# facebook/winterfell

Measured on NVIDIA H100. Metric: prover_ms, lower is better.
Workload: dtype u64

## Files before the change

winterfell_b200/csrc/gl64.cuh:

```cuda
#pragma once
#ifdef __CUDACC_RTC__
typedef unsigned long long uint64_t;
typedef unsigned int uint32_t;
typedef unsigned char uint8_t;
#else
#include <stdint.h>
#endif

#ifdef __CUDACC__
#define GL_HD __host__ __device__ __forceinline__
#else
#define GL_HD inline
#endif

typedef uint64_t u64;
typedef uint32_t u32;
typedef uint8_t u8;

#define GL_P 0xffffffff00000001ULL
#define GL_EPS 0xffffffffULL
#define GL_GENERATOR 7ULL
#define GL_TWO_ADIC_ROOT 7277203076849721926ULL

static inline u64 gl_add_host(u64 a, u64 b) {
    u64 r = a + b;
    if (r < a || r >= GL_P) r += GL_EPS;
    return r;
}
static inline u64 gl_sub_host(u64 a, u64 b) {
    u64 r = a - b;
    if (a < b) r -= GL_EPS;
    return r;
}
static inline u64 gl_reduce128_host(u64 lo, u64 hi) {
    u64 hh = hi >> 32, hl = hi & GL_EPS;
    u64 t = lo - hh;
    if (lo < hh) t -= GL_EPS;
    u64 m = (hl << 32) - hl;
    u64 r = t + m;
    if (r < m) r += GL_EPS;
    if (r >= GL_P) r -= GL_P;
    return r;
}

#if defined(__CUDACC__) && !defined(GL_LITERAL_EPS)
static __constant__ u32 GL_EPS_CONST = 0xffffffffu;
#define GL_EPS_OPERAND , "r"(GL_EPS_CONST)
#define GL_EPSM(n) "%" #n
#else
#define GL_EPS_OPERAND
#define GL_EPSM(n) "0xffffffff"
#endif
#ifdef __CUDA_ARCH__
__device__ __forceinline__ u64 gl_sub(u64 a, u64 b) {
    u64 r;
    asm("{\n\t"
        ".reg .u32 a0, a1, b0, b1, m;\n\t"
        "mov.b64 {a0, a1}, %1;\n\t"
        "mov.b64 {b0, b1}, %2;\n\t"
        "sub.cc.u32 a0, a0, b0;\n\t"
        "subc.cc.u32 a1, a1, b1;\n\t"
        "subc.u32 m, 0, 0;\n\t"
        "sub.cc.u32 a0, a0, m;\n\t"
        "subc.u32 a1, a1, 0;\n\t"
        "mov.b64 %0, {a0, a1};\n\t"
        "}"
        : "=l"(r)
        : "l"(a), "l"(b));
    return r;
}
__device__ __forceinline__ u64 gl_add(u64 a, u64 b) {
    u64 r;
    asm("{\n\t"
        ".reg .u32 a0, a1, b0, b1, m;\n\t"
        "mov.b64 {a0, a1}, %1;\n\t"
        "mov.b64 {b0, b1}, %2;\n\t"
        "sub.cc.u32 b0, 1, b0;\n\t"
        "subc.u32 b1, 0xffffffff, b1;\n\t"
        "sub.cc.u32 a0, a0, b0;\n\t"
        "subc.cc.u32 a1, a1, b1;\n\t"
        "subc.u32 m, 0, 0;\n\t"
        "sub.cc.u32 a0, a0, m;\n\t"
        "subc.u32 a1, a1, 0;\n\t"
        "mov.b64 %0, {a0, a1};\n\t"
        "}"
        : "=l"(r)
        : "l"(a), "l"(b));
    return r;
}
__device__ __forceinline__ void gl_butterfly(u64& a, u64& b) {
    u64 s, d;
    asm("{\n\t"
        ".reg .u32 a0, a1, b0, b1, n0, n1, s0, s1, m;\n\t"
        "mov.b64 {a0, a1}, %2;\n\t"
        "mov.b64 {b0, b1}, %3;\n\t"
        "sub.cc.u32 n0, 1, b0;\n\t"
        "subc.u32 n1, 0xffffffff, b1;\n\t"
        "sub.cc.u32 s0, a0, n0;\n\t"
        "subc.cc.u32 s1, a1, n1;\n\t"
        "subc.u32 m, 0, 0;\n\t"
        "sub.cc.u32 s0, s0, m;\n\t"
        "subc.u32 s1, s1, 0;\n\t"
        "mov.b64 %0, {s0, s1};\n\t"
        "sub.cc.u32 a0, a0, b0;\n\t"
        "subc.cc.u32 a1, a1, b1;\n\t"
        "subc.u32 m, 0, 0;\n\t"
        "sub.cc.u32 a0, a0, m;\n\t"
        "subc.u32 a1, a1, 0;\n\t"
        "mov.b64 %1, {a0, a1};\n\t"
        "}"
        : "=l"(s), "=l"(d)
        : "l"(a), "l"(b));
    a = s;
    b = d;
}
__device__ __forceinline__ u64 gl_canon(u64 r) {
    u64 o;
    asm("{\n\t"
        ".reg .u32 r0, r1, t0, t1, k;\n\t"
        "mov.b64 {r0, r1}, %1;\n\t"
        "add.cc.u32 t0, r0, 0xffffffff;\n\t"
        "addc.cc.u32 t1, r1, 0;\n\t"
        "addc.u32 k, 0, 0;\n\t"
        "sub.u32 r0, r0, k;\n\t"
        "add.u32 r1, r1, k;\n\t"
        "mov.b64 %0, {r0, r1};\n\t"
        "}"
        : "=l"(o)
        : "l"(r));
    return o;
}
__device__ __forceinline__ u64 gl_reduce128(u64 lo, u64 hi) {
    u64 r;
    asm("{\n\t"
        ".reg .u32 c0, c1, c2, c3, k, m, t0, t1;\n\t"
        "mov.b64 {c0, c1}, %1;\n\t"
        "mov.b64 {c2, c3}, %2;\n\t"
        "sub.cc.u32 c0, c0, c3;\n\t"
        "subc.cc.u32 c1, c1, 0;\n\t"
        "subc.u32 m, 0, 0;\n\t"
        "sub.cc.u32 c0, c0, m;\n\t"
        "subc.u32 c1, c1, 0;\n\t"
        "mad.lo.cc.u32 c0, c2, " GL_EPSM(3) ", c0;\n\t"
        "madc.hi.cc.u32 c1, c2, " GL_EPSM(3) ", c1;\n\t"
        "addc.u32 k, 0, 0;\n\t"
        "add.cc.u32 t0, c0, 0xffffffff;\n\t"
        "addc.cc.u32 t1, c1, 0;\n\t"
        "addc.u32 k, k, 0;\n\t"
        "mad.lo.cc.u32 c0, k, " GL_EPSM(3) ", c0;\n\t"
        "madc.hi.u32 c1, k, " GL_EPSM(3) ", c1;\n\t"
        "mov.b64 %0, {c0, c1};\n\t"
        "}"
        : "=l"(r)
        : "l"(lo), "l"(hi) GL_EPS_OPERAND);
    return r;
}
__device__ __forceinline__ u64 gl_mul(u64 a, u64 b) {
    u64 r;
    asm("{\n\t"
        ".reg .u32 a0, a1, b0, b1, c0, c1, c2, c3, o0, o1, o2, k, m, t0, t1;\n\t"
        "mov.b64 {a0, a1}, %1;\n\t"
        "mov.b64 {b0, b1}, %2;\n\t"
        "mul.lo.u32 c0, a0, b0;\n\t"
        "mul.hi.u32 c1, a0, b0;\n\t"
        "mul.lo.u32 c2, a1, b1;\n\t"
        "mul.hi.u32 c3, a1, b1;\n\t"
        "mul.lo.u32 o0, a0, b1;\n\t"
        "mul.hi.u32 o1, a0, b1;\n\t"
        "mad.lo.cc.u32 o0, a1, b0, o0;\n\t"
        "madc.hi.cc.u32 o1, a1, b0, o1;\n\t"
        "addc.u32 o2, 0, 0;\n\t"
        "add.cc.u32 c1, c1, o0;\n\t"
        "addc.cc.u32 c2, c2, o1;\n\t"
        "addc.u32 c3, c3, o2;\n\t"
        "sub.cc.u32 c0, c0, c3;\n\t"
        "subc.cc.u32 c1, c1, 0;\n\t"
        "subc.u32 m, 0, 0;\n\t"
        "sub.cc.u32 c0, c0, m;\n\t"
        "subc.u32 c1, c1, 0;\n\t"
        "mad.lo.cc.u32 c0, c2, " GL_EPSM(3) ", c0;\n\t"
        "madc.hi.cc.u32 c1, c2, " GL_EPSM(3) ", c1;\n\t"
        "addc.u32 k, 0, 0;\n\t"
        "add.cc.u32 t0, c0, 0xffffffff;\n\t"
        "addc.cc.u32 t1, c1, 0;\n\t"
        "addc.u32 k, k, 0;\n\t"
        "mad.lo.cc.u32 c0, k, " GL_EPSM(3) ", c0;\n\t"
        "madc.hi.u32 c1, k, " GL_EPSM(3) ", c1;\n\t"
        "mov.b64 %0, {c0, c1};\n\t"
        "}"
        : "=l"(r)
        : "l"(a), "l"(b) GL_EPS_OPERAND);
    return r;
}
__device__ __forceinline__ u64 gl_mul_weak(u64 a, u64 b) {
    u64 r;
    asm("{\n\t"
        ".reg .u32 a0, a1, b0, b1, c0, c1, c2, c3, o0, o1, o2, k, m;\n\t"
        "mov.b64 {a0, a1}, %1;\n\t"
        "mov.b64 {b0, b1}, %2;\n\t"
        "mul.lo.u32 c0, a0, b0;\n\t"
        "mul.hi.u32 c1, a0, b0;\n\t"
        "mul.lo.u32 c2, a1, b1;\n\t"
        "mul.hi.u32 c3, a1, b1;\n\t"
        "mul.lo.u32 o0, a0, b1;\n\t"
        "mul.hi.u32 o1, a0, b1;\n\t"
        "mad.lo.cc.u32 o0, a1, b0, o0;\n\t"
        "madc.hi.cc.u32 o1, a1, b0, o1;\n\t"
        "addc.u32 o2, 0, 0;\n\t"
        "add.cc.u32 c1, c1, o0;\n\t"
        "addc.cc.u32 c2, c2, o1;\n\t"
        "addc.u32 c3, c3, o2;\n\t"
        "sub.cc.u32 c0, c0, c3;\n\t"
        "subc.cc.u32 c1, c1, 0;\n\t"
        "subc.u32 m, 0, 0;\n\t"
        "sub.cc.u32 c0, c0, m;\n\t"
        "subc.u32 c1, c1, 0;\n\t"
        "mad.lo.cc.u32 c0, c2, " GL_EPSM(3) ", c0;\n\t"
        "madc.hi.cc.u32 c1, c2, " GL_EPSM(3) ", c1;\n\t"
        "addc.u32 k, 0, 0;\n\t"
        "mad.lo.cc.u32 c0, k, " GL_EPSM(3) ", c0;\n\t"
        "madc.hi.u32 c1, k, " GL_EPSM(3) ", c1;\n\t"
        "mov.b64 %0, {c0, c1};\n\t"
        "}"
        : "=l"(r)
        : "l"(a), "l"(b) GL_EPS_OPERAND);
    return r;
}
__device__ __forceinline__ u64 gl_sqr_weak(u64 a) {
    u64 r;
    asm("{\n\t"
        ".reg .u32 a0, a1, c0, c1, c2, c3, o0, o1, o2, k, m;\n\t"
        ".reg .u64 w;\n\t"
        "mov.b64 {a0, a1}, %1;\n\t"
        "mul.wide.u32 w, a0, a0;\n\t"
        "mov.b64 {c0, c1}, w;\n\t"
        "mul.wide.u32 w, a1, a1;\n\t"
        "mov.b64 {c2, c3}, w;\n\t"
        "mul.wide.u32 w, a0, a1;\n\t"
        "mov.b64 {o0, o1}, w;\n\t"
        "add.cc.u32 o0, o0, o0;\n\t"
        "addc.cc.u32 o1, o1, o1;\n\t"
        "addc.u32 o2, 0, 0;\n\t"
        "add.cc.u32 c1, c1, o0;\n\t"
        "addc.cc.u32 c2, c2, o1;\n\t"
        "addc.u32 c3, c3, o2;\n\t"
        "sub.cc.u32 c0, c0, c3;\n\t"
        "subc.cc.u32 c1, c1, 0;\n\t"
        "subc.u32 m, 0, 0;\n\t"
        "sub.cc.u32 c0, c0, m;\n\t"
        "subc.u32 c1, c1, 0;\n\t"
        "mad.lo.cc.u32 c0, c2, " GL_EPSM(2) ", c0;\n\t"
        "madc.hi.cc.u32 c1, c2, " GL_EPSM(2) ", c1;\n\t"
        "addc.u32 k, 0, 0;\n\t"
        "mad.lo.cc.u32 c0, k, " GL_EPSM(2) ", c0;\n\t"
        "madc.hi.u32 c1, k, " GL_EPSM(2) ", c1;\n\t"
        "mov.b64 %0, {c0, c1};\n\t"
        "}"
        : "=l"(r)
        : "l"(a) GL_EPS_OPERAND);
    return r;
}
template <int K>
__device__ __forceinline__ u64 gl_shl_dev(u64 x) {
    constexpr int R = K & 31;
    const u32 x0 = (u32)x, x1 = (u32)(x >> 32);
    const u32 y0 = x0 << R, y1 = R ? __funnelshift_l(x0, x1, R) : x1, y2 = R ? (x1 >> ((32 - R) & 31)) : 0;
    u64 o;
    if (K < 32) {
        asm("{\n\t"
            ".reg .u32 r0, r1, k, t0, t1;\n\t"
            "mad.lo.cc.u32 r0, %3, " GL_EPSM(4) ", %1;\n\t"
            "madc.hi.cc.u32 r1, %3, " GL_EPSM(4) ", %2;\n\t"
            "addc.u32 k, 0, 0;\n\t"
            "add.cc.u32 t0, r0, 0xffffffff;\n\t"
            "addc.cc.u32 t1, r1, 0;\n\t"
            "addc.u32 k, k, 0;\n\t"
            "mad.lo.cc.u32 r0, k, " GL_EPSM(4) ", r0;\n\t"
            "madc.hi.u32 r1, k, " GL_EPSM(4) ", r1;\n\t"
            "mov.b64 %0, {r0, r1};\n\t"
            "}" : "=l"(o) : "r"(y0), "r"(y1), "r"(y2) GL_EPS_OPERAND);
    } else if (K < 64) {
        asm("{\n\t"
            ".reg .u32 r0, r1, k, m, t0, t1;\n\t"
            "sub.cc.u32 r0, 0, %3;\n\t"
            "subc.cc.u32 r1, %1, 0;\n\t"
            "subc.u32 m, 0, 0;\n\t"
            "sub.cc.u32 r0, r0, m;\n\t"
            "subc.u32 r1, r1, 0;\n\t"
            "mad.lo.cc.u32 r0, %2, " GL_EPSM(4) ", r0;\n\t"
            "madc.hi.cc.u32 r1, %2, " GL_EPSM(4) ", r1;\n\t"
            "addc.u32 k, 0, 0;\n\t"
            "add.cc.u32 t0, r0, 0xffffffff;\n\t"
            "addc.cc.u32 t1, r1, 0;\n\t"
            "addc.u32 k, k, 0;\n\t"
            "mad.lo.cc.u32 r0, k, " GL_EPSM(4) ", r0;\n\t"
            "madc.hi.u32 r1, k, " GL_EPSM(4) ", r1;\n\t"
            "mov.b64 %0, {r0, r1};\n\t"
            "}" : "=l"(o) : "r"(y0), "r"(y1), "r"(y2) GL_EPS_OPERAND);
    } else {
        asm("{\n\t"
            ".reg .u32 m0, m1, b;\n\t"
            "mul.lo.u32 m0, %1, " GL_EPSM(4) ";\n\t"
            "mul.hi.u32 m1, %1, " GL_EPSM(4) ";\n\t"
            "sub.cc.u32 m0, m0, %2;\n\t"
            "subc.cc.u32 m1, m1, %3;\n\t"
            "subc.u32 b, 0, 0;\n\t"
            "sub.cc.u32 m0, m0, b;\n\t"
            "subc.u32 m1, m1, 0;\n\t"
            "mov.b64 %0, {m0, m1};\n\t"
            "}" : "=l"(o) : "r"(y0), "r"(y1), "r"(y2) GL_EPS_OPERAND);
    }
    return o;
}
#else
GL_HD u64 gl_add(u64 a, u64 b) { return gl_add_host(a, b); }
GL_HD u64 gl_sub(u64 a, u64 b) { return gl_sub_host(a, b); }
GL_HD u64 gl_reduce128(u64 lo, u64 hi) { return gl_reduce128_host(lo, hi); }
GL_HD u64 gl_mul(u64 a, u64 b) {
    unsigned __int128 x = (unsigned __int128)a * b;
    return gl_reduce128((u64)x, (u64)(x >> 64));
}
GL_HD u64 gl_mul_weak(u64 a, u64 b) { return gl_mul(a, b); }
GL_HD u64 gl_sqr_weak(u64 a) { return gl_mul(a, a); }
static inline void gl_butterfly(u64& a, u64& b) {
    u64 s = gl_add(a, b);
    b = gl_sub(a, b);
    a = s;
}
#endif
#ifdef __CUDACC__
struct GlAcc {
    u32 w0, w1, w2, w3, w4;
};
__device__ __forceinline__ GlAcc acc_zero() { return GlAcc{0, 0, 0, 0, 0}; }
__device__ __forceinline__ void acc_mad(GlAcc& a, u64 x, u64 y) {
    asm("{\n\t"
        ".reg .u32 x0, x1, y0, y1, m0, m1, m2;\n\t"
        "mov.b64 {x0, x1}, %5;\n\t"
        "mov.b64 {y0, y1}, %6;\n\t"
        "mul.lo.u32 m0, x0, y1;\n\t"
        "mul.hi.u32 m1, x0, y1;\n\t"
        "mad.lo.cc.u32 m0, x1, y0, m0;\n\t"
        "madc.hi.cc.u32 m1, x1, y0, m1;\n\t"
        "addc.u32 m2, 0, 0;\n\t"
        "mad.lo.cc.u32 %0, x0, y0, %0;\n\t"
        "madc.hi.cc.u32 %1, x0, y0, %1;\n\t"
        "madc.lo.cc.u32 %2, x1, y1, %2;\n\t"
        "madc.hi.cc.u32 %3, x1, y1, %3;\n\t"
        "addc.u32 %4, %4, 0;\n\t"
        "add.cc.u32 %1, %1, m0;\n\t"
        "addc.cc.u32 %2, %2, m1;\n\t"
        "addc.cc.u32 %3, %3, m2;\n\t"
        "addc.u32 %4, %4, 0;\n\t"
        "}"
        : "+r"(a.w0), "+r"(a.w1), "+r"(a.w2), "+r"(a.w3), "+r"(a.w4)
        : "l"(x), "l"(y));
}
__device__ __forceinline__ u64 acc_reduce(const GlAcc& a) {
    const u64 t = gl_reduce128((u64)a.w0 | ((u64)a.w1 << 32), (u64)a.w2 | ((u64)a.w3 << 32));
    return gl_sub(t, (u64)a.w4 << 32);
}
#endif
GL_HD u64 gl_neg(u64 a) { return a ? GL_P - a : 0; }
GL_HD u64 gl_dbl(u64 a) { return gl_add(a, a); }
GL_HD u64 gl_sqr(u64 a) { return gl_mul(a, a); }

template <int K>
GL_HD u64 gl_mul_2exp(u64 x) {
    if (K == 0) return x;
    if (K == 96) return gl_neg(x);
#ifdef __CUDA_ARCH__
    return gl_shl_dev<K>(x);
#else
    if (K < 64) return gl_reduce128(x << (K & 63), x >> ((64 - K) & 63));
    u64 yl = x << ((K - 64) & 63), yh = (K == 64) ? 0 : (x >> ((128 - K) & 63));
    u64 r = gl_reduce128(0, yl);
    return gl_sub(r, gl_reduce128(yh << 32, 0));
#endif
}

GL_HD u64 gl_pow(u64 a, u64 e) {
    u64 r = 1;
    while (e) {
        if (e & 1) r = gl_mul(r, a);
        a = gl_mul(a, a);
        e >>= 1;
    }
    return r;
}
GL_HD u64 gl_sqr_n(u64 a, int n) {
    for (int i = 0; i < n; i++) a = gl_sqr(a);
    return a;
}
GL_HD u64 gl_inv(u64 x) {
    u64 e2 = gl_mul(gl_sqr(x), x);
    u64 e4 = gl_mul(gl_sqr_n(e2, 2), e2);
    u64 e8 = gl_mul(gl_sqr_n(e4, 4), e4);
    u64 e16 = gl_mul(gl_sqr_n(e8, 8), e8);
    u64 e24 = gl_mul(gl_sqr_n(e16, 8), e8);
    u64 e28 = gl_mul(gl_sqr_n(e24, 4), e4);
    u64 e30 = gl_mul(gl_sqr_n(e28, 2), e2);
    u64 e31 = gl_mul(gl_sqr(e30), x);
    u64 a2 = gl_sqr(e31);
    u64 b = gl_mul(a2, x);
    return gl_mul(gl_sqr_n(a2, 32), b);
}
GL_HD u64 gl_root_of_unity(u32 log_n) { return gl_pow(GL_TWO_ADIC_ROOT, 1ULL << (32 - log_n)); }
GL_HD u64 gl_from_mont(u64 m) { return gl_mul(m, 18446744065119617025ULL); }
GL_HD u64 gl_to_mont(u64 x) { return gl_mul(x, GL_EPS); }

template <int D>
struct GlExt {
    u64 v[D];
};

template <int D>
GL_HD GlExt<D> ext_zero() {
    GlExt<D> r;
#pragma unroll
    for (int i = 0; i < D; i++) r.v[i] = 0;
    return r;
}
template <int D>
GL_HD GlExt<D> ext_from_base(u64 b) {
    GlExt<D> r = ext_zero<D>();
    r.v[0] = b;
    return r;
}
template <int D>
GL_HD GlExt<D> ext_add(const GlExt<D>& a, const GlExt<D>& b) {
    GlExt<D> r;
#pragma unroll
    for (int i = 0; i < D; i++) r.v[i] = gl_add(a.v[i], b.v[i]);
    return r;
}
template <int D>
GL_HD GlExt<D> ext_sub(const GlExt<D>& a, const GlExt<D>& b) {
    GlExt<D> r;
#pragma unroll
    for (int i = 0; i < D; i++) r.v[i] = gl_sub(a.v[i], b.v[i]);
    return r;
}
template <int D>
GL_HD GlExt<D> ext_mul_base(const GlExt<D>& a, u64 b) {
    GlExt<D> r;
#pragma unroll
    for (int i = 0; i < D; i++) r.v[i] = gl_mul(a.v[i], b);
    return r;
}
GL_HD GlExt<1> ext_mul(const GlExt<1>& a, const GlExt<1>& b) {
    GlExt<1> r;
    r.v[0] = gl_mul(a.v[0], b.v[0]);
    return r;
}
GL_HD GlExt<2> ext_mul(const GlExt<2>& a, const GlExt<2>& b) {
    GlExt<2> r;
    u64 a0b0 = gl_mul(a.v[0], b.v[0]);
    r.v[0] = gl_sub(a0b0, gl_dbl(gl_mul(a.v[1], b.v[1])));
    r.v[1] = gl_sub(gl_mul(gl_add(a.v[0], a.v[1]), gl_add(b.v[0], b.v[1])), a0b0);
    return r;
}
GL_HD GlExt<3> ext_mul(const GlExt<3>& a, const GlExt<3>& b) {
    GlExt<3> r;
    u64 a0b0 = gl_mul(a.v[0], b.v[0]), a1b1 = gl_mul(a.v[1], b.v[1]), a2b2 = gl_mul(a.v[2], b.v[2]);
    u64 s01 = gl_mul(gl_add(a.v[0], a.v[1]), gl_add(b.v[0], b.v[1]));
    u64 s02 = gl_mul(gl_add(a.v[0], a.v[2]), gl_add(b.v[0], b.v[2]));
    u64 s12 = gl_mul(gl_add(a.v[1], a.v[2]), gl_add(b.v[1], b.v[2]));
    u64 m = gl_sub(a0b0, a1b1);
    r.v[0] = gl_sub(gl_add(s12, m), a2b2);
    r.v[1] = gl_sub(gl_sub(gl_add(s01, s12), gl_dbl(a1b1)), a0b0);
    r.v[2] = gl_sub(s02, m);
    return r;
}
GL_HD GlExt<1> ext_frobenius(const GlExt<1>& x) { return x; }
GL_HD GlExt<2> ext_frobenius(const GlExt<2>& x) {
    GlExt<2> r;
    r.v[0] = gl_add(x.v[0], x.v[1]);
    r.v[1] = gl_neg(x.v[1]);
    return r;
}
GL_HD GlExt<3> ext_frobenius(const GlExt<3>& x) {
    GlExt<3> r;
    r.v[0] = gl_add(x.v[0], gl_add(gl_mul(10615703402128488253ULL, x.v[1]), gl_mul(6700183068485440220ULL, x.v[2])));
    r.v[1] = gl_add(gl_mul(10050274602728160328ULL, x.v[1]), gl_mul(14531223735771536287ULL, x.v[2]));
    r.v[2] = gl_add(gl_mul(11746561000929144102ULL, x.v[1]), gl_mul(8396469466686423992ULL, x.v[2]));
    return r;
}
GL_HD GlExt<1> ext_inv(const GlExt<1>& a) {
    GlExt<1> r;
    r.v[0] = gl_inv(a.v[0]);
    return r;
}
GL_HD GlExt<2> ext_inv(const GlExt<2>& a) {
    if ((a.v[0] | a.v[1]) == 0) return a;
    GlExt<2> num = ext_frobenius(a);
    GlExt<2> norm = ext_mul(a, num);
    return ext_mul_base(num, gl_inv(norm.v[0]));
}
GL_HD GlExt<3> ext_inv(const GlExt<3>& a) {
    if ((a.v[0] | a.v[1] | a.v[2]) == 0) return a;
    GlExt<3> c1 = ext_frobenius(a);
    GlExt<3> c2 = ext_frobenius(c1);
    GlExt<3> num = ext_mul(c1, c2);
    GlExt<3> norm = ext_mul(a, num);
    return ext_mul_base(num, gl_inv(norm.v[0]));
}
template <int D>
GL_HD GlExt<D> ext_pow(GlExt<D> a, u64 e) {
    GlExt<D> r = ext_from_base<D>(1);
    while (e) {
        if (e & 1) r = ext_mul(r, a);
        a = ext_mul(a, a);
        e >>= 1;
    }
    return r;
}
```

winterfell_b200/csrc/ntt2.cu:

```cuda
#include "minidft.cuh"
#include "ntt.cuh"

#ifndef NTT2_THREADS
#define NTT2_THREADS 256
#endif
#ifndef NTT2_MINB
#define NTT2_MINB 2
#endif
#define NTT2_TILE_ELEMS 8192

template <int LOGS>
struct Plan {
    static constexpr int rounds = LOGS >= 9 ? 3 : 2;
    static constexpr int r0 = (LOGS == 8) ? 4 : 3;
    static constexpr int r1 = (LOGS == 11 || LOGS == 8 || LOGS == 7) ? 4 : 3;
    static constexpr int r2 = LOGS >= 9 ? LOGS - r0 - r1 : 0;
    static_assert(LOGS >= 6 && LOGS <= 11, "plan covers 2^6 .. 2^11");
    static_assert(r0 + r1 + r2 == LOGS && (rounds == 2 || (r2 == 3 || r2 == 4)), "radices must add up");
    static constexpr int lanes = LOGS == 11 ? 4 : 8;
    static constexpr int tw0_entries = 1 << LOGS;
    static constexpr int tw1_entries = rounds == 3 ? (1 << (LOGS - r0)) : 0;
    static constexpr int tw_entries = tw0_entries + tw1_entries;
};
template <int LOGS> __host__ __device__ constexpr int plan_radix(int k) { return k == 0 ? Plan<LOGS>::r0 : (k == 1 ? Plan<LOGS>::r1 : Plan<LOGS>::r2); }
template <int LOGS> __host__ __device__ constexpr int plan_stage(int k) { return k == 0 ? 0 : (k == 1 ? Plan<LOGS>::r0 : Plan<LOGS>::r0 + Plan<LOGS>::r1); }

template <int LK>
__host__ __device__ constexpr u32 swz_const(u32 r) {
    u32 x = r >> LK, h = 0;
    while (x) { h ^= x & ((1u << LK) - 1); x >>= LK; }
    return h;
}
template <int LK>
__device__ __forceinline__ u32 swz_hash(u32 r) {
    if (LK == 1) return __popc(r >> 1) & 1;
    u32 x = r >> 2;
    x ^= x >> 4;
    x ^= x >> 8;
    x ^= x >> 2;
    return x & 3;
}
template <int LK>
__device__ __forceinline__ u32 prow(u32 r) { return r ^ swz_hash<LK>(r); }

__device__ __forceinline__ void bulk_init(u64* mbar, int tid) {
    if (tid == 0) {
        u32 mb = (u32)__cvta_generic_to_shared(mbar);
        asm volatile("mbarrier.init.shared::cta.b64 [%0], 1;" ::"r"(mb));
        asm volatile("fence.mbarrier_init.release.cluster;" ::: "memory");
    }
}
__device__ __forceinline__ void bulk_expect(u64* mbar, u32 bytes) {
    u32 mb = (u32)__cvta_generic_to_shared(mbar);
    asm volatile("mbarrier.arrive.expect_tx.shared::cta.b64 _, [%0], %1;" ::"r"(mb), "r"(bytes) : "memory");
}
__device__ __forceinline__ void bulk_copy(void* smem_dst, const void* gsrc, u32 bytes, u64* mbar) {
    u32 mb = (u32)__cvta_generic_to_shared(mbar), dst = (u32)__cvta_generic_to_shared(smem_dst);
    asm volatile("cp.async.bulk.shared::cluster.global.mbarrier::complete_tx::bytes [%0], [%1], %2, [%3];" ::"r"(dst), "l"(gsrc), "r"(bytes),
                 "r"(mb)
                 : "memory");
}
__device__ __forceinline__ void bulk_wait(u64* mbar) {
    u32 mb = (u32)__cvta_generic_to_shared(mbar), done = 0;
    while (!done)
        asm volatile("{\n\t.reg .pred p;\n\tmbarrier.try_wait.parity.shared::cta.b64 p, [%1], 0;\n\tselp.u32 %0, 1, 0, p;\n\t}" : "=r"(done) : "r"(mb) : "memory");
}

__device__ __forceinline__ void cp_async16(void* smem_dst, const void* gsrc, bool ok) {
    const u32 dst = (u32)__cvta_generic_to_shared(smem_dst);
    asm volatile("cp.async.cg.shared.global [%0], [%1], 16, %2;" ::"r"(dst), "l"(gsrc), "r"(ok ? 16 : 0) : "memory");
}
__device__ __forceinline__ void cp_async8(void* smem_dst, const void* gsrc, bool ok) {
    const u32 dst = (u32)__cvta_generic_to_shared(smem_dst);
    asm volatile("cp.async.ca.shared.global [%0], [%1], 8, %2;" ::"r"(dst), "l"(gsrc), "r"(ok ? 8 : 0) : "memory");
}
__device__ __forceinline__ void cp_async_commit() { asm volatile("cp.async.commit_group;" ::: "memory"); }
__device__ __forceinline__ void cp_async_wait_all() { asm volatile("cp.async.wait_group 0;" ::: "memory"); }

template <int LOGS, int K>
__device__ __forceinline__ void tile_round(u64* __restrict__ s, const u64* __restrict__ tw, const u64* __restrict__ pre, int tid) {
    constexpr int LANES = Plan<LOGS>::lanes, LK = LANES == 8 ? 1 : 2;
    constexpr int R = plan_radix<LOGS>(K), ST = plan_stage<LOGS>(K);
    constexpr int LOGSPAN = LOGS - ST - R;
    constexpr u32 SPAN = 1u << LOGSPAN;
    constexpr bool LAST = LOGSPAN == 0;
    constexpr u32 TASKS = (1u << LOGS) * LANES / 16;
    if (R == 4) {
        for (u32 task = tid; task < TASKS; task += NTT2_THREADS) {
            const u32 lane = task % LANES, bf = task / LANES;
            const u32 lo = bf & (SPAN - 1), base = ((bf >> LOGSPAN) << (LOGSPAN + 4)) + lo;
            const u32 hb = swz_hash<LK>(base);
            u64 x[16];
#pragma unroll
            for (int q = 0; q < 16; q++) {
                const u32 row = (base + ((u32)q << LOGSPAN)) ^ (hb ^ swz_const<LK>((u32)q << LOGSPAN));
                x[q] = s[row * LANES + lane];
            }
            if (K == 0 && pre) {
#pragma unroll
                for (int q = 0; q < 16; q++) x[q] = gl_mul(x[q], __ldg(pre + base + ((u32)q << LOGSPAN)));
            }
            mini_dft<4>(x);
            if (!LAST) {
                const ulonglong2* t2 = reinterpret_cast<const ulonglong2*>(tw + (size_t)lo * 16);
#pragma unroll
                for (int h = 0; h < 8; h++) {
                    const ulonglong2 w = t2[h];
                    if (h > 0) x[2 * h] = gl_mul(x[2 * h], w.x);
                    x[2 * h + 1] = gl_mul(x[2 * h + 1], w.y);
                }
            }
#pragma unroll
            for (int q = 0; q < 16; q++) {
                const u32 row = (base + ((u32)q << LOGSPAN)) ^ (hb ^ swz_const<LK>((u32)q << LOGSPAN));
                s[row * LANES + lane] = x[q];
            }
        }
    } else {
        constexpr int LP = LANES / 2;
        for (u32 task = tid; task < TASKS; task += NTT2_THREADS) {
            const u32 lp = task % LP, bf = task / LP;
            const u32 lo = bf & (SPAN - 1), base = ((bf >> LOGSPAN) << (LOGSPAN + 3)) + lo;
            const u32 hb = swz_hash<LK>(base);
            u64 xa[8], xb[8];
#pragma unroll
            for (int q = 0; q < 8; q++) {
                const u32 row = (base + ((u32)q << LOGSPAN)) ^ (hb ^ swz_const<LK>((u32)q << LOGSPAN));
                const ulonglong2 v = *reinterpret_cast<const ulonglong2*>(s + row * LANES + 2 * lp);
                xa[q] = v.x;
                xb[q] = v.y;
            }
            if (K == 0 && pre) {
#pragma unroll
                for (int q = 0; q < 8; q++) {
                    const u64 f = __ldg(pre + base + ((u32)q << LOGSPAN));
                    xa[q] = gl_mul(xa[q], f);
                    xb[q] = gl_mul(xb[q], f);
                }
            }
            mini_dft<3>(xa);
            mini_dft<3>(xb);
            if (!LAST) {
                const ulonglong2* t2 = reinterpret_cast<const ulonglong2*>(tw + (size_t)lo * 8);
#pragma unroll
                for (int h = 0; h < 4; h++) {
                    const ulonglong2 w = t2[h];
                    if (h > 0) { xa[2 * h] = gl_mul(xa[2 * h], w.x); xb[2 * h] = gl_mul(xb[2 * h], w.x); }
                    xa[2 * h + 1] = gl_mul(xa[2 * h + 1], w.y);
                    xb[2 * h + 1] = gl_mul(xb[2 * h + 1], w.y);
                }
            }
#pragma unroll
            for (int q = 0; q < 8; q++) {
                const u32 row = (base + ((u32)q << LOGSPAN)) ^ (hb ^ swz_const<LK>((u32)q << LOGSPAN));
                *reinterpret_cast<ulonglong2*>(s + row * LANES + 2 * lp) = make_ulonglong2(xa[q], xb[q]);
            }
        }
    }
}

template <int MODE, int LOGS>
__global__ void __launch_bounds__(NTT2_THREADS, NTT2_MINB) ntt2_pass_kernel(const NttPassParams p) {
    extern __shared__ __align__(16) u64 smem[];
    constexpr int LANES = Plan<LOGS>::lanes, LK = LANES == 8 ? 1 : 2, LP = LANES / 2;
    constexpr u32 S = 1u << LOGS;
    const int tid = threadIdx.x;
    const int W = p.W, logW = 31 - __clz(W);
    const int T = W >= LANES ? 1 : (LANES >> logW);
    const int chunks = W >= LANES ? W / LANES : 1;
    u64* s = smem;
    u64* rtw = s + (size_t)S * LANES;
    u64* ctw = rtw + Plan<LOGS>::tw_entries;
    u64* mbar = ctw + (p.has_post ? (size_t)S * T : 0);

    const bool ymap = p.y_in_out;
    const u32 tc = ymap ? blockIdx.y : blockIdx.x;
    const u32 tile = tc / chunks, q0 = (tc % chunks) * LANES;
    const u32 g = ymap ? blockIdx.z : blockIdx.y, b = ymap ? blockIdx.x : blockIdx.z;
    const u32 R = 1u << p.logR, C = 1u << p.logC;
    const u32 ncols = MODE == NTT_STRIDED ? C : R;

    {
        const u64* in = p.in + (size_t)g * p.in_seg_stride + (size_t)b * p.in_batch_stride;
        const u32 lp = tid % LP;
        const u32 l0 = 2 * lp;
        const u32 t0 = W >= LANES ? 0 : (l0 >> logW), t1 = W >= LANES ? 0 : ((l0 + 1) >> logW);
        const u32 w0 = W >= LANES ? q0 + l0 : (l0 & (W - 1)), w1 = W >= LANES ? q0 + l0 + 1 : ((l0 + 1) & (W - 1));
        const u32 c0 = tile * T + t0, c1 = tile * T + t1;
        const bool ok0 = c0 < ncols, ok1 = c1 < ncols;
        const bool yin = MODE == NTT_CONTIG && ymap;
        const u64 istride = MODE == NTT_STRIDED ? ((u64)W << p.logC) : (yin ? ((u64)p.out_row_mul << p.logR) * p.out_W : (u64)W);
        const u64* a0 = MODE == NTT_STRIDED ? in + (size_t)c0 * W + w0
                        : yin ? in + ((size_t)c0 * p.out_row_mul + (size_t)b * p.out_row_add) * p.out_W + p.out_col0 + w0
                              : in + (((size_t)c0 << p.logC) * W + w0);
        const u64* a1 = MODE == NTT_STRIDED ? in + (size_t)c1 * W + w1
                        : yin ? in + ((size_t)c1 * p.out_row_mul + (size_t)b * p.out_row_add) * p.out_W + p.out_col0 + w1
                              : in + (((size_t)c1 << p.logC) * W + w1);
        if (!ok0) a0 = p.in;
        if (!ok1) a1 = p.in;
        const u64 s0 = ok0 ? istride : 0, s1 = ok1 ? istride : 0;
        const bool vec = p.vec_in;
        constexpr u32 ROWS_PER_IT = NTT2_THREADS / LP;
#pragma unroll 4
        for (u32 i = tid / LP; i < S; i += ROWS_PER_IT) {
            u64* dst = s + prow<LK>(i) * LANES + l0;
            if (vec) {
                cp_async16(dst, a0 + i * s0, ok0);
            } else {
                cp_async8(dst, a0 + i * s0, ok0);
                cp_async8(dst + 1, a1 + i * s1, ok1);
            }
        }
        cp_async_commit();
    }

    bulk_init(mbar, tid);
    __syncthreads();
    if (tid == 0) {
        bulk_expect(mbar, Plan<LOGS>::tw_entries * 8);
        bulk_copy(rtw, p.sub_tw, Plan<LOGS>::tw_entries * 8, mbar);
    }

    if (p.has_post && T == 1) {
        const u32 M = 1u << p.logM, lo_mask = (1u << p.tw_split) - 1, c = tile;
        auto wpow = [&](u64 e64) {
            u32 e = (u32)(e64 & (M - 1));
            if (p.inverse && e) e = M - e;
            return gl_mul(p.tw_hi[e >> p.tw_split], p.tw_lo[e & lo_mask]);
        };
        u64 K = wpow((u64)(p.batch0 + b) * p.b_mul * c);
        if (p.ctab) K = gl_mul(K, p.ctab[c < ncols ? c : 0]);
        if (p.cconst != 1) K = gl_mul(K, p.cconst);
        const u64 step = wpow((u64)NTT2_THREADS * p.a_mul * c);
        u64 x = gl_mul(K, wpow((u64)tid * p.a_mul * c));
        for (u32 j = tid; j < S; j += NTT2_THREADS) {
            ctw[j] = x;
            x = gl_mul(x, step);
        }
    } else if (p.has_post) {
        const u32 M = 1u << p.logM, lo_mask = (1u << p.tw_split) - 1;
        for (u32 idx = tid; idx < S * (u32)T; idx += NTT2_THREADS) {
            const u32 j = idx / T, tt = idx % T, c = tile * T + tt;
            u64 e64 = ((u64)j * p.a_mul + (u64)(p.batch0 + b) * p.b_mul) * c;
            u32 e = (u32)(e64 & (M - 1));
            if (p.inverse && e) e = M - e;
            u64 x = gl_mul(p.tw_hi[e >> p.tw_split], p.tw_lo[e & lo_mask]);
            if (p.ctab) x = gl_mul(x, p.ctab[c < ncols ? c : 0]);
            if (p.cconst != 1) x = gl_mul(x, p.cconst);
            ctw[idx] = x;
        }
    }

    cp_async_wait_all();
    bulk_wait(mbar);
    __syncthreads();

    tile_round<LOGS, 0>(s, rtw, p.pre_tab ? p.pre_tab + (size_t)b * p.pre_batch_stride : nullptr, tid);
    __syncthreads();
    if (Plan<LOGS>::rounds == 3) {
        tile_round<LOGS, 1>(s, rtw + Plan<LOGS>::tw0_entries, nullptr, tid);
        __syncthreads();
        tile_round<LOGS, 2>(s, nullptr, nullptr, tid);
    } else {
        tile_round<LOGS, 1>(s, nullptr, nullptr, tid);
    }
    __syncthreads();

    u64* out = p.out + (size_t)g * p.out_seg_stride + (size_t)b * p.out_batch_stride;
    {
        const u32 lp = tid % LP, l0 = 2 * lp;
        const u32 t0 = W >= LANES ? 0 : (l0 >> logW), t1 = W >= LANES ? 0 : ((l0 + 1) >> logW);
        const u32 w0 = W >= LANES ? q0 + l0 : (l0 & (W - 1)), w1 = W >= LANES ? q0 + l0 + 1 : ((l0 + 1) & (W - 1));
        const u32 c0 = tile * T + t0, c1 = tile * T + t1;
        const bool ok0 = c0 < ncols, ok1 = c1 < ncols;
        u64 *o0, *o1, jstride;
        if (MODE == NTT_STRIDED && ymap) {
            o0 = out + (((size_t)c0 << p.logR) * p.out_row_mul + (size_t)b * p.out_row_add) * p.out_W + p.out_col0 + w0;
            o1 = out + (((size_t)c1 << p.logR) * p.out_row_mul + (size_t)b * p.out_row_add) * p.out_W + p.out_col0 + w1;
            jstride = (u64)p.out_row_mul * p.out_W;
        } else if (MODE == NTT_STRIDED) {
            o0 = out + (size_t)c0 * W + w0;
            o1 = out + (size_t)c1 * W + w1;
            jstride = (u64)W << p.logC;
        } else {
            o0 = out + ((size_t)c0 * p.out_row_mul + (size_t)b * p.out_row_add) * p.out_W + p.out_col0 + w0;
            o1 = out + ((size_t)c1 * p.out_row_mul + (size_t)b * p.out_row_add) * p.out_W + p.out_col0 + w1;
            jstride = ((u64)p.out_row_mul << p.logR) * p.out_W;
        }
        const bool post = p.has_post, scale = !p.has_post && p.cconst != 1, vec = p.vec_out;
        const u32 inv_mask = p.inverse ? (S - 1) : 0;
        constexpr u32 ROWS_PER_IT = NTT2_THREADS / LP;
#pragma unroll 4
        for (u32 j = tid / LP; j < S; j += ROWS_PER_IT) {
            const u32 jf = inv_mask ? ((S - j) & inv_mask) : j;
            const u32 r = __brev(jf) >> (32 - LOGS);
            ulonglong2 v = *reinterpret_cast<const ulonglong2*>(s + prow<LK>(r) * LANES + l0);
            if (post) {
                const u64 f0 = ctw[j * T + t0];
                v.x = gl_mul(v.x, f0);
                v.y = gl_mul(v.y, t1 == t0 ? f0 : ctw[j * T + t1]);
            } else if (scale) {
                v.x = gl_mul(v.x, p.cconst);
                v.y = gl_mul(v.y, p.cconst);
            }
            if (vec) {
                if (ok0) *reinterpret_cast<ulonglong2*>(o0 + (u64)j * jstride) = v;
            } else {
                if (ok0) o0[(u64)j * jstride] = v.x;
                if (ok1) o1[(u64)j * jstride] = v.y;
            }
        }
    }
}

template <int LOGS>
__global__ void ntt2_build_tw_kernel(u64* out, u64 w_s) {
    const u32 idx = blockIdx.x * blockDim.x + threadIdx.x;
    if (idx >= (u32)Plan<LOGS>::tw_entries) return;
    int k = idx < (u32)Plan<LOGS>::tw0_entries ? 0 : 1;
    const u32 li = k == 0 ? idx : idx - Plan<LOGS>::tw0_entries;
    const int r = plan_radix<LOGS>(k), st = plan_stage<LOGS>(k);
    const u32 lo = li >> r, qo = li & ((1u << r) - 1);
    const u32 e = (lo * (__brev(qo) >> (32 - r))) << st;
    out[idx] = gl_pow(w_s, e);
}

template <int LOGS>
static size_t smem_bytes_t(const NttPassParams& p) {
    const int lanes = Plan<LOGS>::lanes;
    const size_t S = (size_t)1 << LOGS, T = p.W >= lanes ? 1 : lanes / p.W;
    return (S * lanes + Plan<LOGS>::tw_entries + (p.has_post ? S * T : 0) + 2) * 8;
}
template <int MODE, int LOGS>
static cudaError_t launch_t(const NttPassParams& p, u32 n_segments, u32 n_batch, cudaStream_t st) {
    const int lanes = Plan<LOGS>::lanes;
    const u32 T = p.W >= lanes ? 1 : lanes / p.W, chunks = p.W >= lanes ? p.W / lanes : 1;
    const u32 ncols = MODE == NTT_STRIDED ? (1u << p.logC) : (1u << p.logR);
    const size_t smem = smem_bytes_t<LOGS>(p);
    const u32 tiles = ((ncols + T - 1) / T) * chunks;
    const dim3 grid = p.y_in_out ? dim3(n_batch, tiles, n_segments) : dim3(tiles, n_segments, n_batch);
    cudaError_t e = cudaFuncSetAttribute(ntt2_pass_kernel<MODE, LOGS>, cudaFuncAttributeMaxDynamicSharedMemorySize, (int)smem);
    if (e != cudaSuccess) return e;
    ntt2_pass_kernel<MODE, LOGS><<<grid, NTT2_THREADS, smem, st>>>(p);
    return cudaGetLastError();
}
template <int MODE>
static cudaError_t launch_m(const NttPassParams& p, u32 n_segments, u32 n_batch, cudaStream_t st) {
    switch (p.logS) {
        case 6: return launch_t<MODE, 6>(p, n_segments, n_batch, st);
        case 7: return launch_t<MODE, 7>(p, n_segments, n_batch, st);
        case 8: return launch_t<MODE, 8>(p, n_segments, n_batch, st);
        case 9: return launch_t<MODE, 9>(p, n_segments, n_batch, st);
        case 10: return launch_t<MODE, 10>(p, n_segments, n_batch, st);
        case 11: return launch_t<MODE, 11>(p, n_segments, n_batch, st);
    }
    return cudaErrorInvalidValue;
}
cudaError_t ntt2_launch_pass(int mode, const NttPassParams& p, u32 n_segments, u32 n_batch, cudaStream_t st) {
    return mode == NTT_STRIDED ? launch_m<NTT_STRIDED>(p, n_segments, n_batch, st) : launch_m<NTT_CONTIG>(p, n_segments, n_batch, st);
}
size_t ntt2_tw_entries(int logS) {
    switch (logS) {
        case 6: return Plan<6>::tw_entries; case 7: return Plan<7>::tw_entries; case 8: return Plan<8>::tw_entries;
        case 9: return Plan<9>::tw_entries; case 10: return Plan<10>::tw_entries; case 11: return Plan<11>::tw_entries;
    }
    return 0;
}
cudaError_t ntt2_build_tw(int logS, u64* d_out, cudaStream_t st) {
    const u64 w = gl_root_of_unity((u32)logS);
    const unsigned nb = (unsigned)((ntt2_tw_entries(logS) + 255) / 256);
    switch (logS) {
        case 6: ntt2_build_tw_kernel<6><<<nb, 256, 0, st>>>(d_out, w); break;
        case 7: ntt2_build_tw_kernel<7><<<nb, 256, 0, st>>>(d_out, w); break;
        case 8: ntt2_build_tw_kernel<8><<<nb, 256, 0, st>>>(d_out, w); break;
        case 9: ntt2_build_tw_kernel<9><<<nb, 256, 0, st>>>(d_out, w); break;
        case 10: ntt2_build_tw_kernel<10><<<nb, 256, 0, st>>>(d_out, w); break;
        case 11: ntt2_build_tw_kernel<11><<<nb, 256, 0, st>>>(d_out, w); break;
        default: return cudaErrorInvalidValue;
    }
    return cudaGetLastError();
}
```

Baseline: 114.9.

## Precompute swizzled shared-memory row pointers and unroll bit-reversed output rows in NTT

Shared-memory addresses in the NTT tile rounds are now built from a few per-task base pointers plus compile-time offsets, replacing a per-element XOR-swizzle computation. A fully unrolled output path for forward, vectorized, single-T writes uses compile-time bit-reversed row offsets instead of computing __brev per row. The butterfly's addition is rewritten as a direct add with an epsilon correction, and the reduction helper uses mul.wide. The aim is to cut integer address arithmetic and instruction count, at the cost of more code size and register pressure from the full unrolling.

```diff
diff --git a/winterfell_b200/csrc/gl64.cuh b/winterfell_b200/csrc/gl64.cuh
--- a/winterfell_b200/csrc/gl64.cuh
+++ b/winterfell_b200/csrc/gl64.cuh
@@ -91,16 +91,17 @@
 __device__ __forceinline__ void gl_butterfly(u64& a, u64& b) {
     u64 s, d;
     asm("{\n\t"
-        ".reg .u32 a0, a1, b0, b1, n0, n1, s0, s1, m;\n\t"
+        ".reg .u32 a0, a1, b0, b1, s0, s1, t0, t1, k, m;\n\t"
         "mov.b64 {a0, a1}, %2;\n\t"
         "mov.b64 {b0, b1}, %3;\n\t"
-        "sub.cc.u32 n0, 1, b0;\n\t"
-        "subc.u32 n1, 0xffffffff, b1;\n\t"
-        "sub.cc.u32 s0, a0, n0;\n\t"
-        "subc.cc.u32 s1, a1, n1;\n\t"
-        "subc.u32 m, 0, 0;\n\t"
-        "sub.cc.u32 s0, s0, m;\n\t"
-        "subc.u32 s1, s1, 0;\n\t"
+        "add.cc.u32 s0, a0, b0;\n\t"
+        "addc.cc.u32 s1, a1, b1;\n\t"
+        "addc.u32 k, 0, 0;\n\t"
+        "add.cc.u32 t0, s0, 0xffffffff;\n\t"
+        "addc.cc.u32 t1, s1, 0;\n\t"
+        "addc.u32 k, k, 0;\n\t"
+        "mad.lo.cc.u32 s0, k, " GL_EPSM(4) ", s0;\n\t"
+        "madc.hi.u32 s1, k, " GL_EPSM(4) ", s1;\n\t"
         "mov.b64 %0, {s0, s1};\n\t"
         "sub.cc.u32 a0, a0, b0;\n\t"
         "subc.cc.u32 a1, a1, b1;\n\t"
@@ -110,7 +111,7 @@
         "mov.b64 %1, {a0, a1};\n\t"
         "}"
         : "=l"(s), "=l"(d)
-        : "l"(a), "l"(b));
+        : "l"(a), "l"(b) GL_EPS_OPERAND);
     a = s;
     b = d;
 }
@@ -300,8 +301,9 @@
     } else {
         asm("{\n\t"
             ".reg .u32 m0, m1, b;\n\t"
-            "mul.lo.u32 m0, %1, " GL_EPSM(4) ";\n\t"
-            "mul.hi.u32 m1, %1, " GL_EPSM(4) ";\n\t"
+            ".reg .u64 w;\n\t"
+            "mul.wide.u32 w, %1, " GL_EPSM(4) ";\n\t"
+            "mov.b64 {m0, m1}, w;\n\t"
             "sub.cc.u32 m0, m0, %2;\n\t"
             "subc.cc.u32 m1, m1, %3;\n\t"
             "subc.u32 b, 0, 0;\n\t"
diff --git a/winterfell_b200/csrc/ntt2.cu b/winterfell_b200/csrc/ntt2.cu
--- a/winterfell_b200/csrc/ntt2.cu
+++ b/winterfell_b200/csrc/ntt2.cu
@@ -32,6 +32,23 @@
     return h;
 }
 template <int LK>
+__host__ __device__ constexpr u32 swz_lo(u32 Q) { return swz_const<LK>(Q) ^ (Q & ((1u << LK) - 1)); }
+template <int LK>
+__host__ __device__ constexpr u32 swz_hi(u32 Q) { return Q & ~((1u << LK) - 1); }
+__host__ __device__ constexpr u32 brev_const(u32 v, int bits) {
+    u32 r = 0;
+    for (int i = 0; i < bits; i++) r |= ((v >> i) & 1u) << (bits - 1 - i);
+    return r;
+}
+template <int LOGS, int LK, u32 STEP, u32 N, u32 IT = 0, class F>
+__device__ __forceinline__ void for_brev_rows(F&& f) {
+    if constexpr (IT < N) {
+        constexpr u32 c = brev_const(IT * STEP, LOGS);
+        f(IT, swz_lo<LK>(c), swz_hi<LK>(c));
+        for_brev_rows<LOGS, LK, STEP, N, IT + 1>(f);
+    }
+}
+template <int LK>
 __device__ __forceinline__ u32 swz_hash(u32 r) {
     if (LK == 1) return __popc(r >> 1) & 1;
     u32 x = r >> 2;
@@ -86,16 +103,17 @@
     constexpr bool LAST = LOGSPAN == 0;
     constexpr u32 TASKS = (1u << LOGS) * LANES / 16;
     if (R == 4) {
+#pragma unroll 1
         for (u32 task = tid; task < TASKS; task += NTT2_THREADS) {
             const u32 lane = task % LANES, bf = task / LANES;
             const u32 lo = bf & (SPAN - 1), base = ((bf >> LOGSPAN) << (LOGSPAN + 4)) + lo;
-            const u32 hb = swz_hash<LK>(base);
+            const u32 bh = base ^ swz_hash<LK>(base);
+            u64* pr[1 << LK];
+#pragma unroll
+            for (int v = 0; v < (1 << LK); v++) pr[v] = s + ((bh ^ v) * LANES + lane);
             u64 x[16];
 #pragma unroll
-            for (int q = 0; q < 16; q++) {
-                const u32 row = (base + ((u32)q << LOGSPAN)) ^ (hb ^ swz_const<LK>((u32)q << LOGSPAN));
-                x[q] = s[row * LANES + lane];
-            }
+            for (int q = 0; q < 16; q++) x[q] = pr[swz_lo<LK>((u32)q << LOGSPAN)][swz_hi<LK>((u32)q << LOGSPAN) * LANES];
             if (K == 0 && pre) {
 #pragma unroll
                 for (int q = 0; q < 16; q++) x[q] = gl_mul(x[q], __ldg(pre + base + ((u32)q << LOGSPAN)));
@@ -111,22 +129,22 @@
                 }
             }
 #pragma unroll
-            for (int q = 0; q < 16; q++) {
-                const u32 row = (base + ((u32)q << LOGSPAN)) ^ (hb ^ swz_const<LK>((u32)q << LOGSPAN));
-                s[row * LANES + lane] = x[q];
-            }
+            for (int q = 0; q < 16; q++) pr[swz_lo<LK>((u32)q << LOGSPAN)][swz_hi<LK>((u32)q << LOGSPAN) * LANES] = x[q];
         }
     } else {
         constexpr int LP = LANES / 2;
+#pragma unroll 1
         for (u32 task = tid; task < TASKS; task += NTT2_THREADS) {
             const u32 lp = task % LP, bf = task / LP;
             const u32 lo = bf & (SPAN - 1), base = ((bf >> LOGSPAN) << (LOGSPAN + 3)) + lo;
-            const u32 hb = swz_hash<LK>(base);
+            const u32 bh = base ^ swz_hash<LK>(base);
+            ulonglong2* pr[1 << LK];
+#pragma unroll
+            for (int v = 0; v < (1 << LK); v++) pr[v] = reinterpret_cast<ulonglong2*>(s + ((bh ^ v) * LANES + 2 * lp));
             u64 xa[8], xb[8];
 #pragma unroll
             for (int q = 0; q < 8; q++) {
-                const u32 row = (base + ((u32)q << LOGSPAN)) ^ (hb ^ swz_const<LK>((u32)q << LOGSPAN));
-                const ulonglong2 v = *reinterpret_cast<const ulonglong2*>(s + row * LANES + 2 * lp);
+                const ulonglong2 v = pr[swz_lo<LK>((u32)q << LOGSPAN)][swz_hi<LK>((u32)q << LOGSPAN) * (LANES / 2)];
                 xa[q] = v.x;
                 xb[q] = v.y;
             }
@@ -151,10 +169,7 @@
                 }
             }
 #pragma unroll
-            for (int q = 0; q < 8; q++) {
-                const u32 row = (base + ((u32)q << LOGSPAN)) ^ (hb ^ swz_const<LK>((u32)q << LOGSPAN));
-                *reinterpret_cast<ulonglong2*>(s + row * LANES + 2 * lp) = make_ulonglong2(xa[q], xb[q]);
-            }
+            for (int q = 0; q < 8; q++) pr[swz_lo<LK>((u32)q << LOGSPAN)][swz_hi<LK>((u32)q << LOGSPAN) * (LANES / 2)] = make_ulonglong2(xa[q], xb[q]);
         }
     }
 }
@@ -290,6 +305,28 @@
         const bool post = p.has_post, scale = !p.has_post && p.cconst != 1, vec = p.vec_out;
         const u32 inv_mask = p.inverse ? (S - 1) : 0;
         constexpr u32 ROWS_PER_IT = NTT2_THREADS / LP;
+        if (!p.inverse && vec && T == 1) {
+            const u32 j0 = tid / LP, r0 = __brev(j0) >> (32 - LOGS), rh = r0 ^ swz_hash<LK>(r0);
+            const ulonglong2* pr[1 << LK];
+#pragma unroll
+            for (int v = 0; v < (1 << LK); v++) pr[v] = reinterpret_cast<const ulonglong2*>(s + ((rh ^ v) * LANES + l0));
+            const u64* cj = ctw + j0;
+            u64* oj = o0 + (u64)j0 * jstride;
+            const u64 ostep = (u64)ROWS_PER_IT * jstride;
+            for_brev_rows<LOGS, LK, ROWS_PER_IT, S / ROWS_PER_IT>([&](u32 it, u32 lo, u32 hi) {
+                ulonglong2 v = pr[lo][hi * (LANES / 2)];
+                if (post) {
+                    const u64 f = cj[it * ROWS_PER_IT];
+                    v.x = gl_mul(v.x, f);
+                    v.y = gl_mul(v.y, f);
+                } else if (scale) {
+                    v.x = gl_mul(v.x, p.cconst);
+                    v.y = gl_mul(v.y, p.cconst);
+                }
+                if (ok0) *reinterpret_cast<ulonglong2*>(oj + it * ostep) = v;
+            });
+            return;
+        }
 #pragma unroll 4
         for (u32 j = tid / LP; j < S; j += ROWS_PER_IT) {
             const u32 jf = inv_mask ? ((S - j) & inv_mask) : j;
```

New measurement: 109.8, median of 6. 4.5% less time.
